# nikhilTkur/Multigrid_dolfinx

Measured on AMD Instinct MI355X. Metric: V-cycles/sec + achieved HBM GB/s, 3D Poisson P1 1024³ DoF, 1/2/4/8 MI355X, higher is better.
Workload: dtype f64; 1 GPU; 3D Poisson P1, 6-level 1024^3 fine grid, 1076890625 DoF, V(50,50) weighted Jacobi omega=0.6667, injection, Q1 prolongation, exact block-LU coarsest solve, explicit zeros pruned (7-point rows); levels=6, dim=3, elements_per_dim=1024, parallelism=single

## Files before the change

multigrid_dolfinx_amd/csrc/mg_capi.hip:

```cpp
#include "../../include/mg_hip.h"
#include "mg_csr_check.h"
#include "mg_kernels.hip.h"
#include "mg_direct.hip.h"
#include "mg_jacobi2.hip.h"
#include "mg_jacobik3d.hip.h"
#include "mg_jacobiblk.hip.h"
#include "mg_lattice.hip.h"
#include "mg_diffusion_mf.hip.h"
#include "mg_diffusion_mf_batch.hip.h"
#include "mg_diffusion_adj.hip.h"
#include "mg_diffusion_flux.hip.h"
#include "mg_diffusion_points.hip.h"
#include "mg_diffusion_kappa.hip.h"
#include "mg_block.hip.h"
#include "mg_nullspace.hip.h"
#include "mg_dense_eig.h"

#include <dlfcn.h>
#include <rccl/rccl.h>

#include <algorithm>
#include <array>
#include <cmath>
#include <cstdio>
// ... 301 lines not shown
    int fuse_block_k = 0, fuse_block_ez = 11;
    int direct_block_rows = 2048;
    int fuse_2d_lines = 0;
    int gen_odd_rows = 0;
    int cls_escape = 1;
    int storage_auto = 1;
    int storage_qbits = 0;
    int use_classes = 1;
    int fuse_sweeps = 1;
    int64_t fuse_min_rows = (int64_t)1 << 24;
    int fuse_segments = 0;
    int fuse_nontemporal = 0;
    int fuse_classes = 1;
    int fuse_plain_shape = 0;
    int fuse_plain = 2;
    int class_sweeps = 1;
    int fuse_k = 5;
    int fuse_k_shape = -1;
    int64_t fuse_k_rim_min_rows = (int64_t)1 << 26;
    int fuse_k_segments = 0;
    int timing_force_form = -1;
    int64_t fuse_k_slab_min_rows = (int64_t)1 << 20;
    int fuse_k_slab_min_sweeps = 4;
    int64_t fuse_k_min_rows = (int64_t)1 << 24;
    int64_t fuse_k_small_rows = (int64_t)1 << 22;
    int64_t fuse_k5_min_rows = (int64_t)1 << 26;
    int64_t fuse_k4_min_rows = 0;
    int fuse_k_nt_store = 0;
    int fuse_k_min_side = 32;
    int fuse_k_tail = 1;
    int fuse_k_small_tiles = 0;
    int fuse_k_load_early = 1;
    int64_t fuse_k_load_early_min_rows = (int64_t)1 << 29;
    int fuse_k_plan = 1;
    std::vector<const void*> large_lds_kernels;
    int fuse_shape = 1;
    int fuse_wi = 0;
    int fuse_even = 0;
    int march_sweeps = 1;
    int64_t march_min_rows = (int64_t)1 << 22;
    int march_shape = 0;
    int64_t fuse_small_2d_rows = 2048;
    int fuse_small = 1;
    int fuse_2d = 1;
    int fuse_2d_k = 5;
    int fuse_xcd_chunk = 32;
    int cls_blocks_per_cu = 4;
    DirectSolver direct;
    DevTemp ptab_count;
    int p1_prolong = 0;
    DevTemp rtab_count;
    DevTemp rtab_off;
    DevTemp rtab_w;
    int rtab_m = 0;
    DevTemp ptab_off;
    DevTemp ptab_w;
    Level mass;
    int mass_level = -1;
    DVector mass_out, diff, uexact;
    int uexact_level = -1;
    int64_t uploads = 0, downloads = 0, graph_replays = 0;
    struct SmootherCount { int64_t launches = 0, sweeps = 0, tail = 0; };
    std::vector<std::array<SmootherCount, MG_PATH_COUNT>> smoother_counts;
    int jk3_tail = 0;
    DevBuf<double> stage;
    std::vector<std::unique_ptr<mg_points>> point_sets;
// ... 1232 lines not shown
int march_plan_slot(const mg_context* c, const Level& L, int K) {
    if (!c->fuse_k_plan || K < 3 || K > 5 || !L.cls || L.cls_escape || is_slab(c, L)) return -1;
    const int shape = jk3_shape_for(c, K, L.ncls, true, L.nloc);
    if (shape == 9) return MARCH_PLAN_SLOT_RIM;
    return shape == 7 || shape == 8 ? (K - 3) * 2 + (shape - 7) : -1;
}

int ensure_march_plan(mg_context* c, Level& L, int K, int slot) {
    Level::MarchPlan& mp = L.plan[slot];
    if (mp.iv) return 0;
    JK3PlanArgs a{};
    a.cls = L.cls; a.clead = L.cls_lead; a.P = L.g.plane; a.nx = L.g.nx; a.ny = L.g.ny; a.nz = L.g.nk; a.cmain = L.cmain;
    const bool rim = slot == MARCH_PLAN_SLOT_RIM;
    const int WI = 64 - 2 * K, HY = rim ? jk3_rim_map<5>::HY : 32 - 2 * K + 2;
    a.ntx = (a.nx + WI - 1) / WI; a.nty = (a.ny + HY - 1) / HY;
    const size_t n = (size_t)a.ntx * a.nty * 16 * 4;
    DevBuf<int> iv;
    MG_TRY(iv.alloc(c, n));
    a.plan = iv;
    if (rim) hipLaunchKernelGGL((jk3_plan_rim<5>), dim3((unsigned)(a.ntx * a.nty)), dim3(16 * WAVE), 0, c->stream, a);
    else with_int<3, 4, 5>(K, [&](auto k) { hipLaunchKernelGGL((jk3_plan<decltype(k)::value, 16, 2>), dim3((unsigned)(a.ntx * a.nty)), dim3(16 * WAVE), 0, c->stream, a); });
    HIP_TRY(hipGetLastError());
    std::vector<int> h(n);
    HIP_TRY(hipMemcpyAsync(h.data(), iv, n * sizeof(int), hipMemcpyDeviceToHost, c->stream));
    HIP_TRY(hipStreamSynchronize(c->stream));
    for (size_t i = 0; i < n; i += 4) {
        if (h[i + 1] > h[i]) { ++mp.waves[0]; mp.planes[0] += h[i + 1] - h[i]; }
        if (h[i + 3] > h[i + 2] && (h[i + 2] != h[i] || h[i + 3] != h[i + 1])) { ++mp.waves[1]; mp.planes[1] += h[i + 3] - h[i + 2]; }
    }
    mp.iv = std::move(iv);
    return 0;
}

template <int K, int NW, int LPW, int WPE = (NW == 12 ? 3 : 2), int TR = 256, bool ESC = false, bool B1 = false, bool RIM = false, bool EARLY = false>
int launch_jacobikc_t(mg_context* c, JK3Args a, bool finest, const JK3Range& zr, int seglen) {
    static_assert(!RIM || (NW == jk3_rim_map<K>::NW && WPE == 4 && !ESC && B1), "shape 9 is shape 8 with another line map");
    static_assert(RIM || !EARLY, "only shape 9 has the variant");
    constexpr int EX = 64, EY = RIM ? jk3_rim_map<K>::EY : NW * LPW, WI = EX - 2 * K, HY = EY - 2 * K + 2;
    a.ntx = (a.nx + WI - 1) / WI;
    a.nty = (a.ny + HY - 1) / HY;
    const int64_t ntile = (int64_t)a.ntx * a.nty;
    constexpr size_t lds = RIM ? jk3r_lds_bytes<K, TR>() : B1 ? jk3b_lds_bytes<K, NW, LPW, TR>() : jk3_lds_bytes<K, NW, LPW, TR, ESC>();
    static_assert(lds <= 160 * 1024, "one CU's LDS");
    a.za0 = zr.za0; a.za1 = zr.za1; a.zb0 = zr.zb0; a.zb1 = zr.zb1;
    const int planes = std::max(0, zr.za1 - zr.za0) + std::max(0, zr.zb1 - zr.zb0);
    if (planes <= 0) return 0;
    a.ta = (int)ntile; a.seglen_b = 1;
    int64_t items = 0;
    if (seglen <= 0) {
        int64_t cus = std::max(1, c->prop.multiProcessorCount) * (int64_t)std::max<size_t>(1, std::min<size_t>(160 * 1024 / lds, (size_t)(4 * WPE / NW)));
        if (c->fuse_k_tail > 1) cus = c->fuse_k_tail;
        const double warm = 1.4 * K;
        int best = 1, best_ta = (int)ntile, best_m = 1;
        double best_cost = 1e300;
        const bool tail = c->fuse_k_tail && zr.zb1 <= zr.zb0;
        for (int n = 1; n <= std::max(1, planes / 8); ++n) {
            const int len = (planes + n - 1) / n;
            const int64_t full = ntile * n / cus;
            int64_t ta = tail ? std::min<int64_t>(ntile, full * cus / n) : ntile;
            if (ta <= 0 || (ntile - ta) * 2 > cus) ta = ntile;
            const int64_t tb = ntile - ta;
            const int m = tb > 0 ? (int)std::max<int64_t>(1, std::min<int64_t>(cus / tb, planes / 4)) : 1;
            const double cost = (double)((ta * n + cus - 1) / cus) * (len + warm) + (tb > 0 ? (planes + m - 1) / m + warm : 0.0);
            if (cost < best_cost) { best_cost = cost; best = n; best_ta = (int)ta; best_m = m; }
        }
        if (c->fuse_k_segments > 0) { best = std::min(c->fuse_k_segments, planes); best_ta = (int)ntile; }
        seglen = (planes + best - 1) / best;
        a.ta = best_ta;
        a.seglen_b = best_ta < ntile ? (planes + best_m - 1) / best_m : 1;
    }
    a.seglen = seglen;
    {
        const int nseg = (std::max(0, zr.za1 - zr.za0) + seglen - 1) / seglen + (std::max(0, zr.zb1 - zr.zb0) + seglen - 1) / seglen;
        items = (int64_t)a.ta * nseg;
        if (a.ta < ntile) items += (ntile - a.ta) * (int64_t)((planes + a.seglen_b - 1) / a.seglen_b);
    }
    a.xcd_chunk = (unsigned)c->fuse_xcd_chunk;
    unsigned grid = 0;
    MG_TRY(tile_grid(items, a.xcd_chunk, &grid));
    a.nitems = (unsigned)items;
    if (a.ncls > TR) return fail("more row classes than this tile shape keeps in LDS");
    void (*kern)(JK3Args) = nullptr;
    if constexpr (ESC) kern = sdia_jacobikc_escape<K, NW, LPW, WPE, TR>;
    else if constexpr (RIM && EARLY) kern = finest ? sdia_jacobikc_finest_rim_early<K, TR> : sdia_jacobikc_rim_early<K, TR>;
    else if constexpr (RIM) kern = finest ? sdia_jacobikc_finest_rim<K, TR> : sdia_jacobikc_rim<K, TR>;
    else if constexpr (B1) kern = finest ? sdia_jacobikc_finest_b1<K, NW, LPW, WPE, TR> : sdia_jacobikc_b1<K, NW, LPW, WPE, TR>;
    else kern = finest ? sdia_jacobikc_finest<K, NW, LPW, WPE, TR> : sdia_jacobikc<K, NW, LPW, WPE, TR>;
    MG_TRY(allow_large_lds(c, reinterpret_cast<const void*>(kern), lds));
    hipLaunchKernelGGL(kern, dim3(grid), dim3(NW * WAVE), lds, c->stream, a);
    HIP_TRY(hipGetLastError());
    c->jk3_tail = a.ta < ntile ? 1 : 0;
    return 0;
}

template <int K>
int launch_jacobikc_k(mg_context* c, const JK3Args& a, bool finest, const JK3Range& zr, int seglen, bool whole) {
    if (a.escape) {
        if constexpr (K >= 3) return launch_jacobikc_t<K, 16, 2, 4, 256, true>(c, a, finest, zr, seglen);
        else return fail("levels with escape rows take three to five sweeps per pass");
    }
    if constexpr (K == 2) {
        return launch_jacobikc_t<K, 12, 4>(c, a, finest, zr, seglen);
    } else {
        int shape = jk3_shape_for(c, K, a.ncls, whole, a.P * a.nz);
        if (shape == 1 && a.ncls <= 64 && K <= 4 && c->fuse_k_small_tiles) {
            constexpr int WI = 64 - 2 * K, HY = 48 - 2 * K + 2;
            if ((int64_t)((a.nx + WI - 1) / WI) * ((a.ny + HY - 1) / HY) < std::max(1, c->prop.multiProcessorCount)) shape = 4;
        }
        switch (shape) {
            case 1: return launch_jacobikc_t<K, 12, 4>(c, a, finest, zr, seglen);
            case 4: return launch_jacobikc_t<K, 8, 3, 4, 64>(c, a, finest, zr, seglen);
            case 7: return launch_jacobikc_t<K, 16, 2, 4>(c, a, finest, zr, seglen);
            case 8: return launch_jacobikc_t<K, 16, 2, 4, 256, false, true>(c, a, finest, zr, seglen);
            case 9: if constexpr (K == 5) {
                        if (c->fuse_k_load_early && a.P * a.nz >= c->fuse_k_load_early_min_rows)
                            return launch_jacobikc_t<K, 16, 2, 4, 64, false, true, true, true>(c, a, finest, zr, seglen);
                        return launch_jacobikc_t<K, 16, 2, 4, 64, false, true, true>(c, a, finest, zr, seglen);
                    } else return fail("tile shape 9 takes five sweeps per pass");
            default: return fail("no such tile shape");
        }
    }
}

int launch_jacobikc(mg_context* c, Level& L, int K, const double* x_rows, const double* f_rows, double* out_rows,
                    const JK3Range* zr = nullptr, int seglen = 0) {
    JK3Args a{};
    a.x = x_rows; a.f = f_rows; a.out = out_rows;
    fill_classes_lead(a, L);
    a.P = L.g.plane; a.nx = L.g.nx; a.ny = L.g.ny; a.nz = L.g.nk; a.omega = c->omega;
    const bool dist = is_slab(c, L);
    a.plo = dist && c->comm.rank > 0 ? K : 0;
    a.phi = dist && c->comm.rank + 1 < c->comm.world ? K : 0;
    if (dist && (L.hd < K || L.cls_halo != 1)) return fail("the level's halos are not prepared for that many sweeps per pass");
    if (L.cls_escape && K > L.esc_kmax) return fail("too many escape rows per tile for that many sweeps per pass");
    a.force_form = c->timing_force_form;
    a.nt_store = c->fuse_k_nt_store;
    if (const int slot = march_plan_slot(c, L, K); slot >= 0 && a.force_form < 0 && !zr) {
        if (!L.plan[slot].iv) {
            hipStreamCaptureStatus st = hipStreamCaptureStatusNone;
            HIP_TRY(hipStreamIsCapturing(c->stream, &st));
            if (st == hipStreamCaptureStatusNone) MG_TRY(ensure_march_plan(c, L, K, slot));
        }
        a.plan = L.plan[slot].iv;
    }
    a.escape = L.cls_escape ? 1 : 0; a.dvals = L.dvals; a.mlead = L.mlead; a.sshift = L.R == 1 ? 6 : (L.R == 2 ? 7 : 8);
    const JK3Range whole{0, L.g.nk, 0, 0};
    c->jk3_tail = 0;
    int rc = 0;
    if (!with_int<2, 3, 4, 5>(K, [&](auto k) { rc = launch_jacobikc_k<decltype(k)::value>(c, a, is_finest(c, L), zr ? *zr : whole, seglen, !dist); }))
        return fail("sweeps per pass must be in 2..5");
    return rc;
}

int check_coloring(mg_context* c, Level& L) {
    MG_TRY(need_stored_rows(c, L, "the colouring check of the Gauss-Seidel smoothers"));
    EllArgs a{};
    a.vals = L.vals; a.cols = L.cols; a.codes = L.codes; a.offsets = L.offsets; a.W = L.W;
    a.nloc = L.nloc; a.lead = L.g.lead; a.dinv = L.dinv; a.color_kind = COLOR_LATTICE9; a.grow0 = L.row0; a.gnx = L.g.nx; a.gny = L.g.ny;
    int* d_flag = reinterpret_cast<int*>(c->partials.get());
    HIP_TRY(hipMemsetAsync(d_flag, 0, sizeof(int), c->stream));
    const dim3 grid(blocks_for(L.nloc, 256)), blk(256);
    if (L.sdia) {
        a.vals = L.dvals; a.mlead = L.mlead;
        for (int t = 0; t < 8; ++t) a.up[t] = L.up[t];
        with_int_else<4, 1, 2>(L.R, [&](auto r) { hipLaunchKernelGGL(sdia_check_coloring<decltype(r)::value>, grid, blk, 0, c->stream, a, L.wu, d_flag); });
    } else {
        with_int_else<4, 1, 2>(L.R, [&](auto r) { hipLaunchKernelGGL(ell_check_coloring<decltype(r)::value>, grid, blk, 0, c->stream, a, L.nslices, d_flag); });
    }
    HIP_TRY(hipGetLastError());
// ... 739 lines not shown
        HIP_TRY(hipGetLastError());
        if (add) MG_TRY(exchange_halo(c, F, F.v));
        return 0;
    }
    const int64_t pairs = (int64_t)((F.g.nx + 1) / 2) * F.g.ny;
    const dim3 grid((unsigned)((pairs + kPlaneBlock - 1) / kPlaneBlock), (unsigned)F.g.nk, 1u);
    with_add_keep(add, keep, [&](auto ad, auto kp) {
        hipLaunchKernelGGL((prolong_correct<decltype(ad)::value, decltype(kp)::value>), grid, dim3(kPlaneBlock), 0, c->stream, C.g, F.g, C.v.base, F.v.base, err);
    });
    HIP_TRY(hipGetLastError());
    if (add) MG_TRY(exchange_halo(c, F, F.v));
    return 0;
}

int zero_doubles(mg_context* c, double* p, size_t count) {
    if (c->capturing && count > 0) {
        const unsigned nb = (unsigned)std::min<size_t>((count + 4 * BLOCK - 1) / (4 * BLOCK), (size_t)8 * std::max(1, c->prop.multiProcessorCount));
        hipLaunchKernelGGL(fill_zero, dim3(std::max(1u, nb)), dim3(BLOCK), 0, c->stream, p, (int64_t)count);
        HIP_TRY(hipGetLastError());
        return 0;
    }
    HIP_TRY(hipMemsetAsync(p, 0, count * sizeof(double), c->stream));
    return 0;
}

int zero_vec(mg_context* c, const Level& L, DVector& v) { return zero_doubles(c, v.base, (size_t)L.xlen); }

int dot_device(mg_context* c, const Level& L, const double* x_rows, const double* y_rows, int slot) {
    const int np = (int)std::min<int64_t>(kMaxParts, std::max<int64_t>(1, (L.nloc + 2 * BLOCK - 1) / (2 * BLOCK)));
    hipLaunchKernelGGL(dot_partial, dim3(np), dim3(BLOCK), 0, c->stream, x_rows, y_rows, L.nloc, c->partials);
    hipLaunchKernelGGL(reduce_partials, dim3(1), dim3(BLOCK), 0, c->stream, c->partials, np, c->scalars + slot);
    HIP_TRY(hipGetLastError());
    if (!L.replicated) MG_TRY(allreduce_sum(c, c->scalars + slot, 1));
    return 0;
}

int norm2(mg_context* c, const Level& L, const double* x_rows, double* out) {
    MG_TRY(dot_device(c, L, x_rows, x_rows, 0));
    HIP_TRY(hipMemcpyAsync(c->h_scalars, c->scalars, sizeof(double), hipMemcpyDeviceToHost, c->stream));
    HIP_TRY(hipStreamSynchronize(c->stream));
    *out = std::sqrt(c->h_scalars[0]);
    return 0;
}

double tridiag_max_eig(const std::vector<double>& d, const std::vector<double>& e) {
    const int n = (int)d.size();
    double lo = 1e300, hi = -1e300;
    for (int i = 0; i < n; ++i) {
        const double r = (i > 0 ? std::fabs(e[(size_t)i - 1]) : 0.0) + (i + 1 < n ? std::fabs(e[(size_t)i]) : 0.0);
        lo = std::min(lo, d[(size_t)i] - r);
        hi = std::max(hi, d[(size_t)i] + r);
    }
    auto below = [&](double x) {
        int k = 0;
        double q = d[0] - x;
        if (q < 0.0) ++k;
        for (int i = 1; i < n; ++i) {
            q = d[(size_t)i] - x - e[(size_t)i - 1] * e[(size_t)i - 1] / (q != 0.0 ? q : 1e-300);
            if (q < 0.0) ++k;
        }
        return k;
    };
    for (int it = 0; it < 2000; ++it) {
        const double mid = 0.5 * (lo + hi);
        if (!(mid > lo && mid < hi)) break;
        if (below(mid) < n) lo = mid; else hi = mid;
// ... 1738 lines not shown

int mg_create(int n_levels, int dim, int device, mg_handle* out) {
    if (!out) return fail("null output handle");
    *out = nullptr;
    if (n_levels < 1 || n_levels > 32) return fail("n_levels must be in 1..32");
    if (dim != 2 && dim != 3) return fail("dim must be 2 or 3");
    int ndev = 0;
    HIP_TRY(hipGetDeviceCount(&ndev));
    if (ndev <= 0) return fail("no HIP device visible: this library has no CPU path");
    if (device < 0 || device >= ndev) return fail("device index out of range");
    HIP_TRY(hipSetDevice(device));
    std::unique_ptr<mg_context, ContextDeleter> owner(new mg_context());
    mg_context* const c = owner.get();
    if (const char* e = std::getenv("MG_COMM_PRIORITY")) c->comm_priority = std::atoi(e) != 0;
    if (const char* e = std::getenv("MG_POINT_GROUP")) c->pt_group = std::min(8, std::max(1, std::atoi(e)));
    c->dim = dim;
    c->nlev = n_levels;
    c->device = device;
    c->L.resize(n_levels);
    c->smoother_counts.resize(n_levels);
    HIP_TRY(hipGetDeviceProperties(&c->prop, device));
    HIP_TRY(hipStreamCreateWithFlags(&c->stream, hipStreamNonBlocking));
    {
        int least = 0, greatest = 0;
        HIP_TRY(hipDeviceGetStreamPriorityRange(&least, &greatest));
        HIP_TRY(hipStreamCreateWithPriority(&c->comm_stream, hipStreamNonBlocking, c->comm_priority ? greatest : least));
    }
    HIP_TRY(hipEventCreateWithFlags(&c->ev_boundary, hipEventDisableTiming));
    HIP_TRY(hipEventCreateWithFlags(&c->ev_halo, hipEventDisableTiming));
    MG_TRY(c->partials.alloc(c, 2 * kMaxParts));
    MG_TRY(c->scalars.alloc(c, 8));
    MG_TRY(c->done.alloc(c, 1));
    HIP_TRY(hipMemsetAsync(c->done, 0, sizeof(int), c->stream));
    HIP_TRY(hipHostMalloc(reinterpret_cast<void**>(&c->h_scalars), 16 * sizeof(double), hipHostMallocDefault));
    *out = owner.release();
    return 0;
}

int mg_destroy(mg_handle c) {
    if (c) ContextDeleter{}(c);
    return 0;
}

int mg_device_info(mg_handle c, char* buf, size_t buflen) {
    if (!c || !buf || buflen == 0) return fail("bad arguments");
    snprintf(buf, buflen, "%s %s %d CUs %.1f GiB", c->prop.name, c->prop.gcnArchName, c->prop.multiProcessorCount,
             (double)c->prop.totalGlobalMem / (1024.0 * 1024.0 * 1024.0));
    return 0;
}

int mg_comm_unique_id(void* id_out, size_t id_bytes) {
    if (!id_out || id_bytes < sizeof(ncclUniqueId)) return fail("id buffer must hold 128 bytes");
    MG_TRY(load_rccl());
    ncclUniqueId id;
    NCCL_TRY(g_rccl.GetUniqueId(&id));
    memcpy(id_out, &id, sizeof(id));
    return 0;
}

int mg_comm_selftest(int device) {
    MG_TRY(load_rccl());
    HIP_TRY(hipSetDevice(device));
    ncclUniqueId id;
    NCCL_TRY(g_rccl.GetUniqueId(&id));
    ncclComm_t comm = nullptr;
    NCCL_TRY(g_rccl.CommInitRank(&comm, 1, id, 0));
// ... 349 lines not shown
        if (value != -1 && value != 1 && value != 4 && (value < 7 || value > 9)) return fail("fuse_k_shape must be 1, 4, 7, 8 or 9, or -1 (by sweeps per pass)");
        c->fuse_k_shape = (int)value;
    } else if (k == "fuse_k_slab_min_rows") {
        c->fuse_k_slab_min_rows = value;
    } else if (k == "fuse_k_slab_min_sweeps") {
        if (value < 2) return fail("fuse_k_slab_min_sweeps must be at least 2");
        c->fuse_k_slab_min_sweeps = (int)value;
    } else if (k == "fuse_k_min_rows") {
        c->fuse_k_min_rows = value;
    } else if (k == "fuse_k_small_rows") {
        c->fuse_k_small_rows = value;
    } else if (k == "fuse_k5_min_rows") {
        c->fuse_k5_min_rows = value;
    } else if (k == "fuse_k_rim_min_rows") {
        c->fuse_k_rim_min_rows = value;
    } else if (k == "fuse_k4_min_rows") {
        c->fuse_k4_min_rows = value;
    } else if (k == "fuse_k_nt_store") {
        c->fuse_k_nt_store = value != 0;
    } else if (k == "fuse_k_min_side") {
        if (value < 16 || value > 32) return fail("fuse_k_min_side must be in 16..32");
        c->fuse_k_min_side = (int)value;
    } else if (k == "fuse_k_tail") {
        if (value < 0) return fail("fuse_k_tail must be >= 0");
        c->fuse_k_tail = (int)value;
    } else if (k == "fuse_k_small_tiles") {
        c->fuse_k_small_tiles = value != 0;
    } else if (k == "fuse_k_load_early") {
        if (value != 0 && value != 1) return fail("fuse_k_load_early must be 0 or 1");
        c->fuse_k_load_early = (int)value;
    } else if (k == "fuse_k_load_early_min_rows") {
        if (value < 0) return fail("fuse_k_load_early_min_rows must be >= 0");
        c->fuse_k_load_early_min_rows = value;
    } else if (k == "fuse_k_plan") {
        c->fuse_k_plan = value != 0;
    } else if (k == "fuse_k_segments") {
        if (value < 0) return fail("fuse_k_segments must be >= 0");
        c->fuse_k_segments = (int)value;
    } else if (k == "fuse_classes") {
        c->fuse_classes = value != 0;
    } else if (k == "fuse_nontemporal") {
        c->fuse_nontemporal = value != 0;
    } else if (k == "fuse_segments") {
        if (value < 0) return fail("fuse_segments must be >= 0");
        c->fuse_segments = (int)value;
    } else if (k == "coarse_direct") {
        c->use_direct = value != 0;
        free_direct(c);
    } else if (k == "pcg_chunk") {
        if (value < 1) return fail("pcg_chunk must be positive");
        c->pcg_chunk = (int)value;
    } else if (k == "mf_batch") {
        if (value < 0 || value > MF_BATCH_MAX) return fail("mf_batch must be in 0.." + std::to_string(MF_BATCH_MAX) + " (0 or 1: never fuse)");
        c->mf_batch = (int)value;
    } else {
        return fail("unknown tuning key " + k);
    }
    return 0;
}

namespace {

int upload_permutation(mg_context* c, Level& L, const int64_t* grid_index, int64_t n_rows) {
    if (!grid_index) return 0;
    std::vector<int> p32((size_t)n_rows);
    std::vector<char> seen((size_t)n_rows, 0);
// ... 953 lines not shown
    Level& L = c->L[level];
    MG_TRY(vec_alloc(c, L, &L.ftrue));
    return upload_vector(c, L, L.ftrue, host);
}

int mg_get_vector(mg_handle c, int level, int which, double* host, int gather) {
    MG_TRY(check_level(c, level));
    if (!host) return fail("null host vector");
    HIP_TRY(hipSetDevice(c->device));
    Level& L = c->L[level];
    DVector* v = pick(L, which);
    if (!v || !v->raw) return fail("vector is not available on this level");
    MG_TRY(ensure_stage(c, L.n_global));
    ++c->downloads;
    const unsigned nb = (unsigned)std::min<int64_t>(4096, (L.n_global + 255) / 256);
    if (gather && is_slab(c, L)) {
        DevBuf<double> full;
        MG_TRY(full.alloc(c, (size_t)L.n_global));
        HIP_TRY(hipMemcpyAsync(full + L.row0, v->rows, (size_t)L.nloc * 8, hipMemcpyDeviceToDevice, c->stream));
        MG_TRY(allgather_planes(c, L.splits, L.g.plane, full));
        hipLaunchKernelGGL(gather_out, dim3(nb), dim3(256), 0, c->stream, full, L.perm, L.n_global, (int64_t)0,
                           L.n_global, (int64_t)0, c->stage);
        HIP_TRY(hipStreamSynchronize(c->stream));
        HIP_TRY(hipMemcpy(host, c->stage, (size_t)L.n_global * 8, hipMemcpyDeviceToHost));
        return 0;
    }
    if (is_slab(c, L)) {
        HIP_TRY(hipMemcpyAsync(c->stage, host, (size_t)L.n_global * 8, hipMemcpyHostToDevice, c->stream));
    }
    hipLaunchKernelGGL(gather_out, dim3(nb), dim3(256), 0, c->stream, v->base, L.perm, L.n_global, L.row0, L.nloc,
                       L.g.lead, c->stage);
    HIP_TRY(hipGetLastError());
    HIP_TRY(hipMemcpyAsync(host, c->stage, (size_t)L.n_global * 8, hipMemcpyDeviceToHost, c->stream));
    HIP_TRY(hipStreamSynchronize(c->stream));
    return 0;
}

int mg_set_vector_device(mg_handle c, int level, int which, const double* dev) {
    if (!c) return fail("null handle");
    if (c->comm.active()) return fail("mg_set_vector_device needs a whole (not slab) handle");
    MG_TRY(check_level(c, level));
    HIP_TRY(hipSetDevice(c->device));
    MG_TRY(need_device_pointer(c, dev, "mg_set_vector_device", "the vector"));
    Level& L = c->L[level];
    DVector* v = pick(L, which);
    if (!v) return fail("unknown vector selector");
    MG_TRY(vec_alloc(c, L, v));
    const unsigned nb = (unsigned)std::min<int64_t>(4096, (L.n_global + 255) / 256);
    hipLaunchKernelGGL(scatter_in, dim3(nb), dim3(256), 0, c->stream, dev, L.perm, L.n_global, L.row0, L.g.lead, L.xlen, v->base);
    HIP_TRY(hipGetLastError());
    HIP_TRY(hipStreamSynchronize(c->stream));
    return 0;
}

int mg_get_vector_device(mg_handle c, int level, int which, double* dev) {
    if (!c) return fail("null handle");
    if (c->comm.active()) return fail("mg_get_vector_device needs a whole (not slab) handle");
    MG_TRY(check_level(c, level));
    HIP_TRY(hipSetDevice(c->device));
    MG_TRY(need_device_pointer(c, dev, "mg_get_vector_device", "the vector"));
    Level& L = c->L[level];
    DVector* v = pick(L, which);
    if (!v || !v->raw) return fail("vector is not available on this level");
    const unsigned nb = (unsigned)std::min<int64_t>(4096, (L.n_global + 255) / 256);
    hipLaunchKernelGGL(gather_out, dim3(nb), dim3(256), 0, c->stream, v->base, L.perm, L.n_global, L.row0, L.nloc, L.g.lead, dev);
    HIP_TRY(hipGetLastError());
    HIP_TRY(hipStreamSynchronize(c->stream));
    return 0;
// ... 1162 lines not shown
                MG_TRY(ki_src.alloc(L.kappa.count() * 8));
                MG_TRY(ki_coarse.alloc((L.kappa.count() / 8) * 8));
                HIP_TRY(hipMemcpyAsync(ki_src.p, L.kappa, L.kappa.count() * 8, hipMemcpyDeviceToDevice, c->stream));
            }
            return launch_kappa_ingest(c, ki_src.as<const double>(), L.kappa, ki_coarse.as<double>(), L.N / 2,
                                       MG_KAPPA_ARITHMETIC);
        }
        if (k == "restrict") return level > 0 ? restrict_to(c, level, c->restriction) : fail("level 0");
        if (k == "prolong") return level > 0 ? prolong(c, level, 1) : fail("level 0");
        if (k == "norm2") return dot_device(c, L, L.v.rows, L.v.rows, 1);
        return fail("unknown kernel " + k);
    };
    const auto counts = c->smoother_counts;
    auto timed = [&]() -> int {
        MG_TRY(once());
        HIP_TRY(hipEventRecord(e0, c->stream));
        for (int r = 0; r < reps; ++r) MG_TRY(once());
        HIP_TRY(hipEventRecord(e1, c->stream));
        return 0;
    };
    const int rc = timed();
    c->smoother_counts = counts;
    MG_TRY(rc);
    HIP_TRY(hipEventSynchronize(e1));
    float ms = 0.f;
    HIP_TRY(hipEventElapsedTime(&ms, e0, e1));
    *avg_ms = (double)ms / reps;
    return 0;
}

int mg_sync(mg_handle c) {
    if (!c) return fail("null handle");
    HIP_TRY(hipSetDevice(c->device));
    HIP_TRY(hipStreamSynchronize(c->stream));
    return 0;
}

int mg_memory_bytes(mg_handle c, int64_t* bytes) {
    if (!c || !bytes) return fail("bad arguments");
    *bytes = c->bytes;
    return 0;
}

}
```

multigrid_dolfinx_amd/csrc/mg_jacobik3d.hip.h:

```cpp
#pragma once
#include "mg_jacobi2.hip.h"
#include <type_traits>

namespace mgk {

struct JK3Args {
    const double* x;
    const double* f;
    double* out;
    const unsigned char* cls;
    const double* ctab;
    int64_t clead, P;
    int ncls, cmain;
    double cm[8];
    double omega;
    int nx, ny, nz;
    int plo, phi;
    int ntx, nty, seglen, za0, za1, zb0, zb1;
    int ta, seglen_b;
    unsigned nitems, xcd_chunk;
    int nt_store;
    int escape;
    const double* dvals;
    int64_t mlead;
    int sshift;
    int force_form;
    const int* plan;
};

__device__ __forceinline__ unsigned jk3_cell_offset(int line, int col, int nx, int ny, int tx0, int xcl, int bias) {
    return 8u * (unsigned)(min(max(line, -2), ny + 1) * nx + tx0 + min(col, xcl) + bias);
}
__device__ __forceinline__ const unsigned char* jk3_class_base(const unsigned char* cls, int64_t clead, int bias) {
    return cls + clead - bias;
}

constexpr int jk3_pool(int K) { return K >= 5 ? 512 : 1024; }

template <int K, int NW, int LPW, int TR> constexpr size_t jk3_lds_doubles() {
    return TR * CLS_W + (size_t)K * (NW * LPW + 2) * 64 + 2 * (64 + 2);
}
template <int K, int NW, int LPW, int TR> constexpr size_t jk3b_lds_doubles() {
    return TR * CLS_W + (size_t)(2 * (K - 1) * (NW * LPW + 1) + 1) * 64;
}
template <int K, int NW, int LPW, int TR> constexpr size_t jk3b_lds_bytes() {
    return sizeof(double) * jk3b_lds_doubles<K, NW, LPW, TR>();
}

template <int K, int NW, int LPW, int TR, bool ESC = false> constexpr size_t jk3_lds_bytes() {
    constexpr size_t base = jk3_lds_doubles<K, NW, LPW, TR>();
    return sizeof(double) * (ESC ? (base + CLS_W - 1) / CLS_W * CLS_W + (size_t)(jk3_pool(K) + 1) * CLS_W : base);
}


template <int K, int EY, int E0> struct jk3_caps {
    static constexpr int of(int l) {
        if (E0 < 0) return K;
        const int ey = E0 + l, a = ey + 1 < EY - ey ? ey + 1 : EY - ey;
        return a < K ? a : K;
    }
// ... 555 lines not shown
void sdia_jacobikc_finest(JK3Args a) {
    jk3_body<K, NW, LPW, TR>(a);
}

template <int K, int NW, int LPW, int WPE, int TR>
__global__ __attribute__((amdgpu_flat_work_group_size(NW * WAVE, NW * WAVE), amdgpu_waves_per_eu(WPE, WPE)))
void sdia_jacobikc_b1(JK3Args a) {
    jk3_body<K, NW, LPW, TR, false, true>(a);
}
template <int K, int NW, int LPW, int WPE, int TR>
__global__ __attribute__((amdgpu_flat_work_group_size(NW * WAVE, NW * WAVE), amdgpu_waves_per_eu(WPE, WPE)))
void sdia_jacobikc_finest_b1(JK3Args a) {
    jk3_body<K, NW, LPW, TR, false, true>(a);
}

template <int K, int NW, int LPW, int WPE, int TR>
__global__ __attribute__((amdgpu_flat_work_group_size(NW * WAVE, NW * WAVE), amdgpu_waves_per_eu(WPE, WPE)))
void sdia_jacobikc_escape(JK3Args a) {
    jk3_body<K, NW, LPW, TR, true>(a);
}

template <int K> struct jk3_rim_map {
    static constexpr int NW = 16, RL = K - 1;
    static constexpr int NLM = RL > 2 ? RL : 2;
    static constexpr int EY = 2 * RL + 2 * (NW - 2), HY = EY - 2 * K + 2, WI = 64 - 2 * K;
    static constexpr int first(int wave) { return wave == 0 ? 0 : wave == NW - 1 ? EY - RL : RL + 2 * (wave - 1); }
    static constexpr int lines(int wave) { return wave == 0 || wave == NW - 1 ? RL : 2; }
};
template <int K, int KIND> struct jk3_rim_kind {
    static constexpr int NL = KIND == 0 ? 2 : K - 1;
    static constexpr int cap(int l) { return KIND == 0 ? K : KIND == 1 ? l + 1 : K - 1 - l; }
};

template <int K, int TR> constexpr size_t jk3r_lds_bytes() {
    return sizeof(double) * (TR * CLS_W + (size_t)(2 * (K - 1) * (jk3_rim_map<K>::EY + 1) + 1) * 64);
}

template <int K, int TR, bool EARLY = false>
__device__ __forceinline__ void jk3_rim_body(const JK3Args& a) {
    using MAP = jk3_rim_map<K>;
    constexpr int EX = 64, NW = MAP::NW, EY = MAP::EY, NCM = MAP::NLM, WI = MAP::WI, HY = MAP::HY;
    constexpr int IS = (EY + 1) * EX, PS = (K - 1) * IS;
    static_assert(CLS_W == 8, "table rows of eight doubles");
    static_assert(K >= 3 && NCM <= 4, "a wave's class bytes of a plane live in one register");
    static_assert(NCM * (K + 1) <= 64, "the fast-path flags live in one scalar register pair");
    static_assert(8 * ((K - 2) * IS + (NCM + 1) * EX) < 65536, "every LDS access of a step is `register + 16-bit immediate`");
    extern __shared__ double j2_smem[];
    double* const sT = j2_smem;
    const int lane = threadIdx.x & 63;
    const int wave = __builtin_amdgcn_readfirstlane((int)(threadIdx.x >> 6));

    unsigned id;
    {
        const unsigned b = blockIdx.x, xcd = b & 7u, j = b >> 3, ch = a.xcd_chunk;
        id = ((j / ch) * 8u + xcd) * ch + (j % ch);
    }
    if (id >= a.nitems) return;
    const unsigned ntile = (unsigned)(a.ntx * a.nty);
    const int nsa = (a.za1 - a.za0 + a.seglen - 1) / a.seglen;
    const int nsb = (a.zb1 - a.zb0 + a.seglen - 1) / a.seglen;
    const unsigned items_a = (unsigned)a.ta * (unsigned)(nsa + max(nsb, 0));
    unsigned tt;
    int z0, z1;
    if (id < items_a) {
        const int seg = (int)(id / (unsigned)a.ta);
        tt = id % (unsigned)a.ta;
        z0 = seg < nsa ? a.za0 + seg * a.seglen : a.zb0 + (seg - nsa) * a.seglen;
        z1 = min(seg < nsa ? a.za1 : a.zb1, z0 + a.seglen);
    } else {
        const unsigned j = id - items_a, tb = ntile - (unsigned)a.ta;
        tt = (unsigned)a.ta + j % tb;
        z0 = a.za0 + (int)(j / tb) * a.seglen_b;
        z1 = min(a.za1, z0 + a.seglen_b);
    }
    const int tiy = (int)(tt / (unsigned)a.ntx), tix = (int)(tt % (unsigned)a.ntx);
    if (z1 <= z0) return;
    const int tx0 = tix * WI - K, ty0 = tiy * HY - (K - 1);

    {
        const int nt = a.ncls * CLS_W;
        for (int i = threadIdx.x; i < nt; i += NW * WAVE) {
            double v = a.ctab[i];
            if ((i & (CLS_W - 1)) == CLS_W - 1) {
                const double d = a.ctab[i - 4];
                v = a.omega * (1.0 / (d != 0.0 ? d : 1.0));
            }
            sT[i] = v;
        }
        constexpr int NZ = (2 * (K - 1) * (EY + 1) + 1) * EX;
        for (int i = threadIdx.x; i < NZ; i += NW * WAVE) sT[TR * CLS_W + i] = 0.0;
    }
    const double m0 = a.cm[0], m1 = a.cm[1], m2 = a.cm[2], m3 = a.cm[3], m4 = a.cm[4], m5 = a.cm[5], m6 = a.cm[6];
    const double mcf = a.omega * (1.0 / (m3 != 0.0 ? m3 : 1.0));
    const int cmain = a.cmain;

    const int ey0 = MAP::first(wave);
    const int wkind = wave == 0 ? 1 : wave == NW - 1 ? 2 : 0;
    int bcur = 0, bprev = 0;
    int lbase = TR * CLS_W + ey0 * EX + lane;
    asm volatile("" : "+v"(lbase));
    auto limg = [&](int base, int t) -> double* { return j2_smem + base + (t - 1) * IS + EX; };
    unsigned inT = 0;
#pragma unroll
    for (int l = 0; l < NCM; ++l) {
        const int ey = ey0 + l;
        if (lane >= K && lane < EX - K && ey >= K - 1 && ey <= EY - K && tx0 + lane < a.nx && ty0 + ey < a.ny) inT |= 1u << l;
    }
    auto shof = [&](int l) -> int {
        const int64_t r = (int64_t)(ty0 + ey0 + l) * a.nx + (tx0 + (lbase & 63));
        return r < 0 ? -1 : (r >= a.P ? 1 : 0);
    };

    const int bias = 2 * a.nx + K + 2;
    const int xcl = a.nx + 1 - tx0;
    unsigned eo[NCM];
#pragma unroll
    for (int l = 0; l < NCM; ++l) {
        eo[l] = jk3_cell_offset(ty0 + ey0 + l, lane, a.nx, a.ny, tx0, xcl, bias);
        asm volatile("" : "+v"(eo[l]));
    }
    const unsigned eos = jk3_cell_offset(ty0 + ey0 - 1, lane, a.nx, a.ny, tx0, xcl, bias);
    const unsigned eon = jk3_cell_offset(ty0 + ey0 + MAP::lines(wave), lane, a.nx, a.ny, tx0, xcl, bias);
    const unsigned char* const clsb = jk3_class_base(a.cls, a.clead, bias);
// ... 203 lines not shown
        using KD = decltype(kind);
        constexpr int NL = KD::NL;
        double x0w[NL], x0e[NL];
        if (t == 1) {
#pragma unroll
            for (int l = 0; l < NL; ++l) { x0w[l] = jk3_from_west(X[l]); x0e[l] = jk3_from_east(X[l]); }
        }
#pragma unroll
        for (int l = 0; l < NL; ++l) {
            if (t > KD::cap(l)) continue;
            const int iw = l * EX;
            double ys, yw, yd, ye, yn;
            if (t == 1) {
                ys = l > 0 ? X[l > 0 ? l - 1 : l] : hS;
                yw = x0w[l]; yd = X[l]; ye = x0e[l];
                yn = l + 1 < NL ? X[l + 1 < NL ? l + 1 : l] : hN;
            } else {
                const double* const img = limg(bcur, t - 1);
                ys = img[iw - EX]; yw = img[iw - 1]; yd = img[iw]; ye = img[iw + 1]; yn = img[iw + EX];
            }
            const dvec2_t* const tr = reinterpret_cast<const dvec2_t*>(sT + CLS_W * cls_now(K - t, l));
            const dvec2_t t01 = tr[0], t23 = tr[1], t45 = tr[2];
            double s = acc[t - 1][l];
            s = fma(t01.y, ys, s);
            s = fma(t23.x, yw, s);
            s = fma(t23.y, yd, s);
            s = fma(t45.x, ye, s);
            s = fma(t45.y, yn, s);
            acc[t - 1][l] = s;
            __builtin_amdgcn_sched_barrier(0);
        }
    };

    auto step = [&](auto kind, const int k) __attribute__((always_inline)) {
        using KD = decltype(kind);
        constexpr int NL = KD::NL;
        constexpr unsigned long long ALLFAST = (1ull << (NL * (K + 1))) - 1ull;
        k_plane = k; k_store = k >= z0;
        bcur = lbase + (k & 1) * PS;
        bprev = lbase + ((k + 1) & 1) * PS;
        asm volatile("" : "+v"(bcur));
        asm volatile("" : "+v"(bprev));
        {
            const unsigned long long u = (unsigned long long)(a.out - bias + (int64_t)k * a.P);
            const unsigned lo = (unsigned)__builtin_amdgcn_readfirstlane((int)(unsigned)u);
            const unsigned hi = (unsigned)__builtin_amdgcn_readfirstlane((int)(unsigned)(u >> 32));
            k_out = (__attribute__((address_space(1))) char*)(((unsigned long long)hi << 32) | lo);
        }
#pragma unroll
        for (int l = 0; l < NL; ++l) asm volatile("" : "+v"(X[l]));
        const bool interior = interior_step(k);
        if (k == khi) {
            unsigned m = 0;
#pragma unroll
            for (int l = 0; l < NL; ++l)
                if (__builtin_amdgcn_readfirstlane((int)(__ballot(cls_of(0, l) != cmain) == 0ull))) m |= 1u << l;
            fast = 0;
#pragma unroll
            for (int j = 0; j < K; ++j) {
                fast |= (unsigned long long)m << (j * NL);
                cw[j] = cw[0];
            }
        }
        int form = kform;
        if (!interior) {
            unsigned m = 0;
// ... 10 lines not shown
            if ((a.plo > 0 || k >= 1) && (a.phi > 0 || k + K + 1 < a.nz)) {
                if (fast == ALLFAST) {
                    form = 0;
                } else {
                    bool same = true;
#pragma unroll
                    for (int j = 1; j <= K; ++j) same = same && cw[j] == cw[0];
                    if (__builtin_amdgcn_readfirstlane((int)(__ballot(!same) == 0ull))) form = 1;
                }
            }
        }
        if (a.force_form >= 0) form = a.force_form;
        if (form == 0) phase_a_fast(std::false_type{}, kind);
        else if (form == 1) phase_a_fast(std::true_type{}, kind);
        else phase_a_general(kind);
#pragma unroll
        for (int l = 0; l < NL; ++l) XP[l] = X[l];
#pragma unroll
        for (int l = 0; l < NL; ++l) {
#pragma unroll
            for (int j = 0; j + 1 < K; ++j) fr[j][l] = fr[j + 1][l];
            if (KD::cap(l) >= 2) asm volatile("" : "+v"(fr[K - 2][l]));
        }
        if (!interior) {
#pragma unroll
            for (int j = 0; j < K; ++j) cw[j] = cw[j + 1];
            fast >>= NL;
        }
        if constexpr (EARLY) {
            __builtin_amdgcn_sched_barrier(0);
            load_f_classes(kind, k + K + 1, k + K, interior_step(k + 1));
            __builtin_amdgcn_sched_barrier(0);
        }
        __syncthreads();
#pragma unroll
        for (int t = 1; t <= K; ++t) {
            if (form == 0) phase_b_fast(std::false_type{}, kind, t);
            else if (form == 1) phase_b_fast(std::true_type{}, kind, t);
            else phase_b_general(kind, t);
            __builtin_amdgcn_sched_barrier(0);
            if constexpr (!EARLY) load_slice(kind, t - 1, K, k + K + 1, k + K, interior_step(k + 1));
            else if (t == 1) load_x(kind, k + K + 1);
            __builtin_amdgcn_sched_barrier(0);
        }
    };

    auto march = [&](auto kind) __attribute__((always_inline)) {
        load_slice(kind, 0, 1, z0 - K, z0 - K - 1, false);
        __syncthreads();
        for (int k = z0 - 2 * K; k < z1; ++k) step(kind, k);
    };
    if (wkind == 0) march(jk3_rim_kind<K, 0>{});
    else if (wkind == 1) march(jk3_rim_kind<K, 1>{});
    else march(jk3_rim_kind<K, 2>{});
}

template <int K, int TR>
__global__ __attribute__((amdgpu_flat_work_group_size(16 * WAVE, 16 * WAVE), amdgpu_waves_per_eu(4, 4)))
void sdia_jacobikc_rim(JK3Args a) {
    jk3_rim_body<K, TR>(a);
}
template <int K, int TR>
__global__ __attribute__((amdgpu_flat_work_group_size(16 * WAVE, 16 * WAVE), amdgpu_waves_per_eu(4, 4)))
void sdia_jacobikc_finest_rim(JK3Args a) {
    jk3_rim_body<K, TR>(a);
}
template <int K, int TR>
__global__ __attribute__((amdgpu_flat_work_group_size(16 * WAVE, 16 * WAVE), amdgpu_waves_per_eu(4, 4)))
void sdia_jacobikc_rim_early(JK3Args a) {
    jk3_rim_body<K, TR, true>(a);
}
template <int K, int TR>
__global__ __attribute__((amdgpu_flat_work_group_size(16 * WAVE, 16 * WAVE), amdgpu_waves_per_eu(4, 4)))
void sdia_jacobikc_finest_rim_early(JK3Args a) {
    jk3_rim_body<K, TR, true>(a);
}

struct JK3WindowArgs {
    const unsigned char* cls;
    int64_t clead, P;
    int nx, ny, nz, ntx, nty;
    unsigned* most;
};

template <int K, int NW, int LPW>
__global__ __launch_bounds__(256) void jk3_escape_window(JK3WindowArgs a) {
    constexpr int EX = 64, EY = NW * LPW, WI = EX - 2 * K, HY = EY - 2 * K + 2, W = K + 2;
    __shared__ unsigned s_ring[W], s_plane;
    const int tiy = (int)(blockIdx.x / (unsigned)a.ntx), tix = (int)(blockIdx.x % (unsigned)a.ntx);
    const int tx0 = tix * WI - K, ty0 = tiy * HY - (K - 1), xcl = a.nx + 1 - tx0;
    unsigned win = 0u, best = 0u;
    for (int p = 0; p < a.nz; ++p) {
        if (threadIdx.x == 0) s_plane = 0u;
        __syncthreads();
        unsigned n = 0u;
        for (int i = threadIdx.x; i < EX * EY; i += 256) {
            const int ex = i % EX, line = ty0 + i / EX;
            if (ex > xcl || line < -2 || line > a.ny + 1) continue;
            const int64_t row = (int64_t)p * a.P + (int64_t)line * a.nx + tx0 + ex;
            n += a.cls[a.clead + row] == CLS_ESCAPE ? 1u : 0u;
        }
        if (n) atomicAdd(&s_plane, n);
        __syncthreads();
        if (threadIdx.x == 0) {
            win += s_plane - (p >= W ? s_ring[p % W] : 0u);
            s_ring[p % W] = s_plane;
            best = max(best, win);
        }
// ... 86 lines not shown
```

Measured before the change: 5.118 V-cycles/s.

## Replace block barrier in rim march kernel with neighbour-wave flag waits

Adds a variant of the shape-9 fused Jacobi march kernel where the per-plane __syncthreads is replaced by LDS flags: each wave publishes its step counter and spins only until the waves above and below have reached it. The aim is to let waves drift apart instead of the whole 16-wave block stalling at every plane. It is used for mid-sized levels (2^26 to 2^29 rows), so at this problem size it applies to the coarser levels rather than the finest. A bounded poll count with an expiry flag, checked on host at sync points, guards against deadlock, at the cost of extra LDS, spin-polling overhead and a host readback on mg_sync.

```diff
diff --git a/multigrid_dolfinx_amd/csrc/mg_capi.hip b/multigrid_dolfinx_amd/csrc/mg_capi.hip
--- a/multigrid_dolfinx_amd/csrc/mg_capi.hip
+++ b/multigrid_dolfinx_amd/csrc/mg_capi.hip
@@ -357,6 +357,10 @@
     int fuse_k_small_tiles = 0;
     int fuse_k_load_early = 1;
     int64_t fuse_k_load_early_min_rows = (int64_t)1 << 29;
+    int fuse_k_wave_sync = 1;
+    int64_t fuse_k_wave_sync_min_rows = (int64_t)1 << 26;
+    int64_t fuse_k_wave_sync_max_rows = (int64_t)1 << 29;
+    DevBuf<int> march_expired;
     int fuse_k_plan = 1;
     std::vector<const void*> large_lds_kernels;
     int fuse_shape = 1;
@@ -1655,15 +1659,17 @@
     return 0;
 }
 
-template <int K, int NW, int LPW, int WPE = (NW == 12 ? 3 : 2), int TR = 256, bool ESC = false, bool B1 = false, bool RIM = false, bool EARLY = false>
+template <int K, int NW, int LPW, int WPE = (NW == 12 ? 3 : 2), int TR = 256, bool ESC = false, bool B1 = false, bool RIM = false, bool EARLY = false,
+          bool WSYNC = false>
 int launch_jacobikc_t(mg_context* c, JK3Args a, bool finest, const JK3Range& zr, int seglen) {
     static_assert(!RIM || (NW == jk3_rim_map<K>::NW && WPE == 4 && !ESC && B1), "shape 9 is shape 8 with another line map");
     static_assert(RIM || !EARLY, "only shape 9 has the variant");
+    static_assert(EARLY || !WSYNC, "the neighbour waits come with the early loads");
     constexpr int EX = 64, EY = RIM ? jk3_rim_map<K>::EY : NW * LPW, WI = EX - 2 * K, HY = EY - 2 * K + 2;
     a.ntx = (a.nx + WI - 1) / WI;
     a.nty = (a.ny + HY - 1) / HY;
     const int64_t ntile = (int64_t)a.ntx * a.nty;
-    constexpr size_t lds = RIM ? jk3r_lds_bytes<K, TR>() : B1 ? jk3b_lds_bytes<K, NW, LPW, TR>() : jk3_lds_bytes<K, NW, LPW, TR, ESC>();
+    constexpr size_t lds = RIM ? jk3r_lds_bytes<K, TR, WSYNC>() : B1 ? jk3b_lds_bytes<K, NW, LPW, TR>() : jk3_lds_bytes<K, NW, LPW, TR, ESC>();
     static_assert(lds <= 160 * 1024, "one CU's LDS");
     a.za0 = zr.za0; a.za1 = zr.za1; a.zb0 = zr.zb0; a.zb1 = zr.zb1;
     const int planes = std::max(0, zr.za1 - zr.za0) + std::max(0, zr.zb1 - zr.zb0);
@@ -1705,6 +1711,7 @@
     if (a.ncls > TR) return fail("more row classes than this tile shape keeps in LDS");
     void (*kern)(JK3Args) = nullptr;
     if constexpr (ESC) kern = sdia_jacobikc_escape<K, NW, LPW, WPE, TR>;
+    else if constexpr (RIM && WSYNC) kern = finest ? sdia_jacobikc_finest_wsync<K, TR> : sdia_jacobikc_wsync<K, TR>;
     else if constexpr (RIM && EARLY) kern = finest ? sdia_jacobikc_finest_rim_early<K, TR> : sdia_jacobikc_rim_early<K, TR>;
     else if constexpr (RIM) kern = finest ? sdia_jacobikc_finest_rim<K, TR> : sdia_jacobikc_rim<K, TR>;
     else if constexpr (B1) kern = finest ? sdia_jacobikc_finest_b1<K, NW, LPW, WPE, TR> : sdia_jacobikc_b1<K, NW, LPW, WPE, TR>;
@@ -1736,7 +1743,10 @@
             case 7: return launch_jacobikc_t<K, 16, 2, 4>(c, a, finest, zr, seglen);
             case 8: return launch_jacobikc_t<K, 16, 2, 4, 256, false, true>(c, a, finest, zr, seglen);
             case 9: if constexpr (K == 5) {
-                        if (c->fuse_k_load_early && a.P * a.nz >= c->fuse_k_load_early_min_rows)
+                        const int64_t rows = a.P * a.nz;
+                        if (c->fuse_k_wave_sync && rows >= c->fuse_k_wave_sync_min_rows && rows < c->fuse_k_wave_sync_max_rows)
+                            return launch_jacobikc_t<K, 16, 2, 4, 64, false, true, true, true, true>(c, a, finest, zr, seglen);
+                        if (c->fuse_k_load_early && rows >= c->fuse_k_load_early_min_rows)
                             return launch_jacobikc_t<K, 16, 2, 4, 64, false, true, true, true>(c, a, finest, zr, seglen);
                         return launch_jacobikc_t<K, 16, 2, 4, 64, false, true, true>(c, a, finest, zr, seglen);
                     } else return fail("tile shape 9 takes five sweeps per pass");
@@ -1758,6 +1768,7 @@
     if (L.cls_escape && K > L.esc_kmax) return fail("too many escape rows per tile for that many sweeps per pass");
     a.force_form = c->timing_force_form;
     a.nt_store = c->fuse_k_nt_store;
+    a.wait_expired = c->march_expired;
     if (const int slot = march_plan_slot(c, L, K); slot >= 0 && a.force_form < 0 && !zr) {
         if (!L.plan[slot].iv) {
             hipStreamCaptureStatus st = hipStreamCaptureStatusNone;
@@ -2563,6 +2574,17 @@
     hipLaunchKernelGGL(reduce_partials, dim3(1), dim3(BLOCK), 0, c->stream, c->partials, np, c->scalars + slot);
     HIP_TRY(hipGetLastError());
     if (!L.replicated) MG_TRY(allreduce_sum(c, c->scalars + slot, 1));
+    return 0;
+}
+
+int sync_and_check_march(mg_context* c) {
+    int* const h = reinterpret_cast<int*>(c->h_scalars + 9);
+    HIP_TRY(hipMemcpyAsync(h, c->march_expired, sizeof(int), hipMemcpyDeviceToHost, c->stream));
+    HIP_TRY(hipStreamSynchronize(c->stream));
+    if (*h) {
+        HIP_TRY(hipMemsetAsync(c->march_expired, 0, sizeof(int), c->stream));
+        return fail("march: a wave's wait expired");
+    }
     return 0;
 }
 
@@ -4367,6 +4389,8 @@
     MG_TRY(c->scalars.alloc(c, 8));
     MG_TRY(c->done.alloc(c, 1));
     HIP_TRY(hipMemsetAsync(c->done, 0, sizeof(int), c->stream));
+    MG_TRY(c->march_expired.alloc(c, 1));
+    HIP_TRY(hipMemsetAsync(c->march_expired, 0, sizeof(int), c->stream));
     HIP_TRY(hipHostMalloc(reinterpret_cast<void**>(&c->h_scalars), 16 * sizeof(double), hipHostMallocDefault));
     *out = owner.release();
     return 0;
@@ -4782,6 +4806,15 @@
     } else if (k == "fuse_k_load_early_min_rows") {
         if (value < 0) return fail("fuse_k_load_early_min_rows must be >= 0");
         c->fuse_k_load_early_min_rows = value;
+    } else if (k == "fuse_k_wave_sync") {
+        if (value != 0 && value != 1) return fail("fuse_k_wave_sync must be 0 or 1");
+        c->fuse_k_wave_sync = (int)value;
+    } else if (k == "fuse_k_wave_sync_min_rows") {
+        if (value < 0) return fail("fuse_k_wave_sync_min_rows must be >= 0");
+        c->fuse_k_wave_sync_min_rows = value;
+    } else if (k == "fuse_k_wave_sync_max_rows") {
+        if (value < 0) return fail("fuse_k_wave_sync_max_rows must be >= 0");
+        c->fuse_k_wave_sync_max_rows = value;
     } else if (k == "fuse_k_plan") {
         c->fuse_k_plan = value != 0;
     } else if (k == "fuse_k_segments") {
@@ -5801,8 +5834,7 @@
                        L.g.lead, c->stage);
     HIP_TRY(hipGetLastError());
     HIP_TRY(hipMemcpyAsync(host, c->stage, (size_t)L.n_global * 8, hipMemcpyDeviceToHost, c->stream));
-    HIP_TRY(hipStreamSynchronize(c->stream));
-    return 0;
+    return sync_and_check_march(c);
 }
 
 int mg_set_vector_device(mg_handle c, int level, int which, const double* dev) {
@@ -7031,8 +7063,7 @@
 int mg_sync(mg_handle c) {
     if (!c) return fail("null handle");
     HIP_TRY(hipSetDevice(c->device));
-    HIP_TRY(hipStreamSynchronize(c->stream));
-    return 0;
+    return sync_and_check_march(c);
 }
 
 int mg_memory_bytes(mg_handle c, int64_t* bytes) {
diff --git a/multigrid_dolfinx_amd/csrc/mg_jacobik3d.hip.h b/multigrid_dolfinx_amd/csrc/mg_jacobik3d.hip.h
--- a/multigrid_dolfinx_amd/csrc/mg_jacobik3d.hip.h
+++ b/multigrid_dolfinx_amd/csrc/mg_jacobik3d.hip.h
@@ -26,6 +26,7 @@
     int sshift;
     int force_form;
     const int* plan;
+    int* wait_expired;
 };
 
 __device__ __forceinline__ unsigned jk3_cell_offset(int line, int col, int nx, int ny, int tx0, int xcl, int bias) {
@@ -647,11 +648,16 @@
     static constexpr int cap(int l) { return KIND == 0 ? K : KIND == 1 ? l + 1 : K - 1 - l; }
 };
 
-template <int K, int TR> constexpr size_t jk3r_lds_bytes() {
-    return sizeof(double) * (TR * CLS_W + (size_t)(2 * (K - 1) * (jk3_rim_map<K>::EY + 1) + 1) * 64);
-}
-
-template <int K, int TR, bool EARLY = false>
+template <int K, int TR, bool WSYNC = false> constexpr size_t jk3r_lds_bytes() {
+    return sizeof(double) * (TR * CLS_W + (size_t)(2 * (K - 1) * (jk3_rim_map<K>::EY + 1) + 1) * 64) +
+           (WSYNC ? sizeof(int) * (jk3_rim_map<K>::NW + 2) : 0);
+}
+constexpr int JK3_WAIT_POLLS = 1 << 23;
+#ifndef JK3_WAIT_SLEEP
+#define JK3_WAIT_SLEEP 1
+#endif
+
+template <int K, int TR, bool EARLY = false, bool WSYNC = false>
 __device__ __forceinline__ void jk3_rim_body(const JK3Args& a) {
     using MAP = jk3_rim_map<K>;
     constexpr int EX = 64, NW = MAP::NW, EY = MAP::EY, NCM = MAP::NLM, WI = MAP::WI, HY = MAP::HY;
@@ -704,6 +710,10 @@
         }
         constexpr int NZ = (2 * (K - 1) * (EY + 1) + 1) * EX;
         for (int i = threadIdx.x; i < NZ; i += NW * WAVE) sT[TR * CLS_W + i] = 0.0;
+        if constexpr (WSYNC) {
+            int* const fl = reinterpret_cast<int*>(sT + TR * CLS_W + NZ);
+            if (threadIdx.x < NW + 2) fl[threadIdx.x] = threadIdx.x == 0 || threadIdx.x == NW + 1 ? 0x7fffffff : 0;
+        }
     }
     const double m0 = a.cm[0], m1 = a.cm[1], m2 = a.cm[2], m3 = a.cm[3], m4 = a.cm[4], m5 = a.cm[5], m6 = a.cm[6];
     const double mcf = a.omega * (1.0 / (m3 != 0.0 ? m3 : 1.0));
@@ -973,6 +983,25 @@
         }
     };
 
+    int* const wflag = reinterpret_cast<int*>(j2_smem + TR * CLS_W + (2 * (K - 1) * (EY + 1) + 1) * EX) + wave;
+    int polls = JK3_WAIT_POLLS;
+    auto wave_sync = [&](const int s) __attribute__((always_inline)) {
+        __hip_atomic_store(wflag + 1, s, __ATOMIC_RELEASE, __HIP_MEMORY_SCOPE_WORKGROUP);
+        for (;;) {
+            const int below = __builtin_amdgcn_readfirstlane(__hip_atomic_load(wflag, __ATOMIC_RELAXED, __HIP_MEMORY_SCOPE_WORKGROUP));
+            const int above = __builtin_amdgcn_readfirstlane(__hip_atomic_load(wflag + 2, __ATOMIC_RELAXED, __HIP_MEMORY_SCOPE_WORKGROUP));
+            if (min(below, above) >= s) break;
+            if (polls <= 0) {
+                if (polls == 0 && lane == 0) *a.wait_expired = 1;
+                polls = -1;
+                break;
+            }
+            --polls;
+            __builtin_amdgcn_s_sleep(JK3_WAIT_SLEEP);
+        }
+        __builtin_amdgcn_fence(__ATOMIC_ACQUIRE, "workgroup");
+    };
+
     auto step = [&](auto kind, const int k) __attribute__((always_inline)) {
         using KD = decltype(kind);
         constexpr int NL = KD::NL;
@@ -1049,7 +1078,8 @@
             load_f_classes(kind, k + K + 1, k + K, interior_step(k + 1));
             __builtin_amdgcn_sched_barrier(0);
         }
-        __syncthreads();
+        if constexpr (WSYNC) wave_sync(k - (z0 - 2 * K) + 1);
+        else __syncthreads();
 #pragma unroll
         for (int t = 1; t <= K; ++t) {
             if (form == 0) phase_b_fast(std::false_type{}, kind, t);
@@ -1091,6 +1121,17 @@
 __global__ __attribute__((amdgpu_flat_work_group_size(16 * WAVE, 16 * WAVE), amdgpu_waves_per_eu(4, 4)))
 void sdia_jacobikc_finest_rim_early(JK3Args a) {
     jk3_rim_body<K, TR, true>(a);
+}
+
+template <int K, int TR>
+__global__ __attribute__((amdgpu_flat_work_group_size(16 * WAVE, 16 * WAVE), amdgpu_waves_per_eu(4, 4)))
+void sdia_jacobikc_wsync(JK3Args a) {
+    jk3_rim_body<K, TR, true, true>(a);
+}
+template <int K, int TR>
+__global__ __attribute__((amdgpu_flat_work_group_size(16 * WAVE, 16 * WAVE), amdgpu_waves_per_eu(4, 4)))
+void sdia_jacobikc_finest_wsync(JK3Args a) {
+    jk3_rim_body<K, TR, true, true>(a);
 }
 
 struct JK3WindowArgs {
```

After: 5.155 V-cycles/s (median of 6 runs). Within noise of the previous version (+0.7%).
